# cbg-ethz/metMHN

Measured on AMD Instinct MI355X. Metric: full-cohort log-lik+grad evals/sec at n=20 events; kronvec HBM GB/s, higher is better.
Workload: dtype f64

## Files before the change

metmhn_amd/csrc/engine.hip:

```cpp
#include <hip/hip_runtime.h>
#include <rccl/rccl.h>
#include <dlfcn.h>

#include <algorithm>
#include <chrono>
#include <cmath>
#include <cstdio>
#include <cstdlib>
#include <cstring>
#include <string>
#include <vector>

#include "../../include/metmhn_amd.h"
#include "kernels.h"
#include "tsolve.h"
#include "small.h"
#include "wsolve.h"
#include "wclass.h"
#include "sampler.h"

namespace mmhn {

static thread_local std::string g_err;

struct Fail {
  std::string msg;
};
#define HIPCHECK(expr)                                                                       \
  do {                                                                                       \
    hipError_t e_ = (expr);                                                                  \
    if (e_ != hipSuccess)                                                                    \
      throw Fail{std::string(#expr) + ": " + hipGetErrorString(e_) + " (" + __FILE__ + ":" + \
                 std::to_string(__LINE__) + ")"};                                            \
  } while (0)
#define REQUIRE(cond, text) \
  do {                      \
    if (!(cond)) throw Fail{std::string(text)}; \
  } while (0)

template <typename U>
struct DevArr {
  U* p = nullptr;
  size_t n = 0;
  void alloc(size_t count) {
    if (count <= n && p) return;
    release();
    if (count == 0) return;
    HIPCHECK(hipMalloc(reinterpret_cast<void**>(&p), count * sizeof(U)));
    n = count;
  }
  void release() {
    if (p) (void)hipFree(p);
    p = nullptr;
    n = 0;
  }
  ~DevArr() { release(); }
  DevArr() = default;
  DevArr(const DevArr&) = delete;
  DevArr& operator=(const DevArr&) = delete;
  DevArr(DevArr&& o) noexcept : p(o.p), n(o.n) { o.p = nullptr; o.n = 0; }
  DevArr& operator=(DevArr&& o) noexcept {
    if (this != &o) { release(); p = o.p; n = o.n; o.p = nullptr; o.n = 0; }
    return *this;
  }
};

struct CList {
  std::vector<CItem> items;
  std::vector<int> deps;
  DevArr<CItem> d_items;
  DevArr<int> d_deps;
  int maxk = 0;
  int nlevels = 0;
  void clear() { items.clear(); deps.clear(); maxk = 0; nlevels = 0; }
};
enum Route : uint8_t { RT_W = 0, RT_P = 1, RT_T = 2 };

struct Staged {
  std::vector<int> pats, paired, probs;
  DevArr<int> d_pats, d_paired, d_probs;
  std::vector<int2> map, lmap;
  std::vector<int> lof;
  DevArr<int2> d_map, d_lmap;
  DevArr<int2> d_grc;
  CList cl[2];
  int maxk = 0;
  bool kind2 = false;
  bool empty() const { return pats.empty(); }
};

struct Batch {
  std::vector<PatRec> pats;
  std::vector<Desc> dJ, dS;
  std::vector<int2> mapJ, mapS;
  long long vecJ = 0, vecS = 0, asize = 0, tabJ = 0, tabS = 0;
  int id = 0;
  int maxkJ = 0, maxkS = 0;
  int maxkcJ = 0;
  bool has_kind2 = false;
  std::vector<int2> lmapJ, lmapS;
  std::vector<int> lofJ, lofS;
  std::vector<int2> mapX;
  DevArr<int2> d_mapX;
  DevArr<int2> d_grc[4];
  DevArr<int2> d_grcJ;
  std::vector<int> sp_list[3][SP_NCLASS];
  DevArr<int> d_sp_list[3][SP_NCLASS];
  bool has_small = false;
  int mk1p = 9;
  Staged stg[2];
  std::vector<int> paired;
  DevArr<int> d_paired;
  std::vector<uint8_t> route;
  std::vector<int> olist;
  DevArr<int> d_olist;
  bool wpath = false;
  bool wdirect = false;
  std::vector<WDesc> wd;
  DevArr<WDesc> d_wd;
  int wnx = -1;
  std::vector<WChain> wchains;
  DevArr<WChain> d_wchains;
  long long offT = 0;
  CList clJ[2];
  std::vector<int2> lmapT;
  std::vector<int> lofT;
  DevArr<int2> d_lmapT;
  int maxkT = 0, maxkP = 0;
  int max_dl = 0;
  std::vector<int> ptoff;
  std::vector<uint32_t> ptiles;
  DevArr<int> d_ptoff;
  DevArr<uint32_t> d_ptiles;
  double seeded_bytes_P = 0;
  std::vector<int4> pcl;
  DevArr<int4> d_pcl;
  DevArr<PatRec> d_pats;
  DevArr<Desc> d_dJ, d_dS;
  DevArr<int2> d_mapJ, d_mapS, d_lmapJ, d_lmapS;
};

static bool dead_tile(const Desc& d, uint32_t H) {
  if (d.mode != JOINT || d.seedbit < TB) return false;
  const uint32_t xhi = H << TB, hmask = ~((1u << TB) - 1u);
  if (xhi & (1u << d.seedbit)) return false;
  if (xhi & d.lone & hmask) return true;
  const uint32_t pp = d.pairP & hmask & ~(1u << 31);
  const uint32_t pm = (pp << 1);
  if (((xhi & pp) << 1) != (xhi & pm)) return true;
  return false;
}

static void build_levels(const std::vector<int2>& map, const std::vector<Desc>* descs, bool prune,
                         std::vector<int2>& lmap, std::vector<int>& lof) {
  int maxl = 0;
  std::vector<int2> keep;
  keep.reserve(map.size());
  for (const int2& m : map) {
    if (prune && descs && dead_tile((*descs)[m.x], (uint32_t)m.y)) continue;
    keep.push_back(m);
    maxl = std::max(maxl, popc((uint32_t)m.y));
  }
  lof.assign(maxl + 2, 0);
  for (const int2& m : keep) lof[popc((uint32_t)m.y) + 1]++;
  for (int l = 0; l <= maxl; ++l) lof[l + 1] += lof[l];
  lmap.resize(keep.size());
  std::vector<int> cur(lof.begin(), lof.end() - 1);
  for (const int2& m : keep) lmap[cur[popc((uint32_t)m.y)]++] = m;
}

static inline long long a_size(const Desc& d) {
  const int kP = popc(d.maskP), kM = popc(d.maskM), kE = popc(d.pairP);
  return ((long long)(kP + 1) << kP) + ((long long)(kM + 1) << kM) + ((long long)(kE + 2) << kE);
}

static void add_tiles(std::vector<int2>& map, int prob, int k) {
  const int tiles = k > TB ? 1 << (k - TB) : 1;
  for (int t = 0; t < tiles; ++t) map.push_back(make_int2(prob, t));
// ... 152 lines not shown
    double v;
    if (e == 0) v = em[0];
    else if (e == 1) v = nm[0];
    else if (e == 2) v = n_em;
    else if (e == 3) v = n_pat;
    else {
      int q = e - 4;
      if (q < NN) v = em[1 + q];
      else if ((q -= NN) < NN) v = nm[1 + q];
      else if ((q -= NN) < N) v = em[1 + NN + q];
      else if ((q -= N) < N) v = nm[1 + NN + q];
      else v = em[1 + NN + N + (q - N)];
    }
    o[e] = v;
  }
}

__global__ void k_pack_wsums(const double* __restrict__ sums, int N, double w, double* __restrict__ o, double flag) {
  const int st = 1 + N * N + 2 * N, NN = N * N;
  if (blockIdx.x == 0 && threadIdx.x == 0) o[st] = flag;
  const double* em = sums;
  const double* nm = sums + st;
  for (int e = blockIdx.x * blockDim.x + threadIdx.x; e < st; e += gridDim.x * blockDim.x)
    o[e] = e < 1 + NN + N ? w * em[e] + nm[e] : w * em[e];
}

__global__ void k_copy_words(const uint4* __restrict__ src, uint4* __restrict__ dst, int n) {
  const int i = blockIdx.x * blockDim.x + threadIdx.x;
  if (i < n) dst[i] = src[i];
}
__global__ void k_begin_eval(const uint4* __restrict__ src, uint4* __restrict__ dst, int n, double* __restrict__ sums, int nsums,
                             uint4* __restrict__ z, long long nz) {
  const long long i0 = (long long)blockIdx.x * blockDim.x + threadIdx.x, step = (long long)gridDim.x * blockDim.x;
  if (i0 < n) dst[i0] = src[i0];
  if (i0 < nsums) sums[i0] = 0.0;
  for (long long i = i0; i < nz; i += step) z[i] = uint4{0u, 0u, 0u, 0u};
}

__global__ __launch_bounds__(BLOCK) void k_reduce_parts_pack(const double* __restrict__ part, int stride, int nelem, int nchunk,
                                                             double* sums, int mode, int N, double a, double b,
                                                             double* __restrict__ o) {
  const int e = blockIdx.x * BLOCK + threadIdx.x;
  if (e == 0 && mode == 2) o[stride] = b;
  if (e >= stride) return;
  double em = sums[e], nm = sums[stride + e];
  if (e < nelem) {
    double acc0 = 0, acc1 = 0;
#pragma unroll 8
    for (int c = 0; c < nchunk; ++c) {
      acc0 += part[((long long)c * 2 + 0) * stride + e];
      acc1 += part[((long long)c * 2 + 1) * stride + e];
    }
    em += acc0; nm += acc1;
    sums[e] = em; sums[stride + e] = nm;
  }
  const int NN = N * N;
  if (mode == 2) { o[e] = e < 1 + NN + N ? a * em + nm : a * em; return; }
  if (e == 0) { o[0] = em; o[1] = nm; o[2] = a; o[3] = b; }
  else if (e < 1 + NN) { o[4 + (e - 1)] = em; o[4 + NN + (e - 1)] = nm; }
  else if (e < 1 + NN + N) { o[4 + 2 * NN + (e - 1 - NN)] = em; o[4 + 2 * NN + N + (e - 1 - NN)] = nm; }
  else o[4 + 2 * NN + 2 * N + (e - 1 - NN - N)] = em;
}

template <typename T>
struct Engine : EngineBase {
  int n = 0, N = 0;
  size_t ws_limit = 0;
  DevArr<Params<T>> d_par;
  Params<T>* h_par = nullptr;
  double* h_abi = nullptr;
  void* h_par_dev = nullptr;
  double* h_abi_dev = nullptr;
  bool zero_copy = true;
  bool time_kernels = true;
  std::vector<int8_t> dat;
  long long n_pat = 0;
  int n_cols = 0;
  std::vector<Batch> batches;
  double n_em = 0;
  DevArr<T> pi, lidgJ, qJ, rhsJ, rhsS, pS, lidgS, qS, seedS, GS, dots, bmJ, bmS, tabJ, tabS;
  DevArr<T> zarena;
  struct View { T* p = nullptr; } GJ, DJ, Abuf;
  static long long zarena_elems(long long nJ, long long asize, int N) { return up4(3 * nJ * N * N) + up4(3 * nJ * N) + up4(asize); }
  static long long up4(long long v) { return (v + 3) / 4 * 4; }
  int pi_owner = -1, qJ_owner = -1;
  DevArr<double> lp, out, sums, abi_sums, redbuf;
  DevArr<JLink<T>> links;
  ncclComm_t comm = nullptr;
  int comm_rank = 0, comm_size = 1;
  DevArr<uint16_t> d_perm;
  DevArr<int> d_lvl;
  bool use_jacobi = false;
  bool poison = false;
  hipStream_t side[3] = {};
  hipEvent_t ev_fork[3] = {}, ev_join[3] = {};
  bool small_path = true;
  int prep_split_max = 2048;
  int psolve_min = 384;
  int wsolve_min = 128;
  bool force_timing = false;
  bool coop_fault = false;
  int pcl_per = 16;
  int coop_wgs = 0;
  bool coop = true;
  DevArr<CoopCtl> coop_ctl;
  DevArr<unsigned> coop_flags[2];
  unsigned coop_epoch = 0;
  int coop_slot = 0;
  int cur_lane = 0;
  unsigned* h_abort = nullptr;
  unsigned* h_abort_dev = nullptr;
  int wsolve_wgs = 0;
  int wsolve_mode = 1;
  DevArr<T> piM, qM;
  int n_cu = 256;
  mmhn_counters cnt{};
  std::vector<std::pair<hipEvent_t, hipEvent_t>> ev_pool;
  size_t ev_used = 0;
  std::vector<double> ev_bytes;
  std::vector<int> ev_slot;

  Engine(int dev, int n_mut) : n(n_mut), N(n_mut + 1) {
    device = dev;
    cnt.comm_rank = -1;
    REQUIRE(n_mut >= 1 && n_mut < MAXN, "n_mut must be in [1, 31]");
    DevGuard guard(device);
    HIPCHECK(hipStreamCreateWithFlags(&stream, hipStreamNonBlocking));
    d_par.alloc(NPSET);
    HIPCHECK(hipHostMalloc(reinterpret_cast<void**>(&h_par), NPSET * sizeof(Params<T>), hipHostMallocDefault));
    HIPCHECK(hipHostGetDevicePointer(&h_par_dev, h_par, 0));
    static_assert(sizeof(Params<T>) % sizeof(uint4) == 0, "parameter block: whole 16-byte words");
    sums.alloc(2 * stride());
    size_t free_b = 0, total_b = 0;
    HIPCHECK(hipMemGetInfo(&free_b, &total_b));
    ws_limit = (size_t)(0.7 * (double)free_b);
    {
      std::vector<uint16_t> perm((size_t)(TB + 1) << TB, 0);
      std::vector<int> lvl((size_t)(TB + 1) * (TB + 2), 0);
      for (int t = 0; t <= TB; ++t) {
        int pos = 0;
        for (int l = 0; l <= t; ++l) {
          lvl[(size_t)t * (TB + 2) + l] = pos;
          for (uint32_t x = 0; x < (1u << t); ++x)
            if (popc(x) == l) perm[((size_t)t << TB) + pos++] = (uint16_t)x;
        }
        lvl[(size_t)t * (TB + 2) + t + 1] = pos;
      }
      d_perm.alloc(perm.size());
      d_lvl.alloc(lvl.size());
      HIPCHECK(hipMemcpy(d_perm.p, perm.data(), perm.size() * sizeof(uint16_t), hipMemcpyHostToDevice));
      HIPCHECK(hipMemcpy(d_lvl.p, lvl.data(), lvl.size() * sizeof(int), hipMemcpyHostToDevice));
      const char* sv = std::getenv("MMHN_SOLVER");
      use_jacobi = sv && std::string(sv) == "jacobi";
      if (const char* pm = std::getenv("MMHN_PSOLVE_MIN")) { psolve_min = std::atoi(pm); wsolve_min = psolve_min; }
      if (const char* pm = std::getenv("MMHN_WSOLVE_MIN")) wsolve_min = std::atoi(pm);
      if (const char* pm = std::getenv("MMHN_COOP")) coop = std::atoi(pm) != 0;
      if (const char* pm = std::getenv("MMHN_TIME_KERNELS")) force_timing = std::atoi(pm) != 0;
      if (const char* pm = std::getenv("MMHN_COOP_WGS")) coop_wgs = std::atoi(pm);
      if (const char* pm = std::getenv("MMHN_PCL_PER")) pcl_per = std::max(1, std::atoi(pm));
      if (const char* pm = std::getenv("MMHN_COOP_FAULT")) coop_fault = std::atoi(pm) != 0;
      if (const char* po = std::getenv("MMHN_POISON")) poison = std::atoi(po) != 0;
      if (const char* sp = std::getenv("MMHN_SMALL")) small_path = std::atoi(sp) != 0;
      if (const char* sp = std::getenv("MMHN_ZEROCOPY")) zero_copy = std::atoi(sp) != 0;
      if (const char* sp = std::getenv("MMHN_PREP_SPLIT")) prep_split_max = std::atoi(sp);
      if (const char* ms = std::getenv("MMHN_WSOLVE")) wsolve_mode = std::atoi(ms);
      if (const char* ms = std::getenv("MMHN_WSOLVE_WGS")) wsolve_wgs = std::atoi(ms);
// ... 633 lines not shown
          }
        }
        auto item_tiles = [&](const int4& it) -> long long {
          if (it.y == 2) return 0;
          const Desc& dj = b.dJ[it.x];
          const int kc = popc(it.y == 0 ? dj.maskP : dj.maskM);
          return (long long)(it.w - it.z) << (kc > PCA ? kc - PCA : 0);
        };
        std::stable_sort(b.pcl.begin(), b.pcl.end(), [&](const int4& x, const int4& y) { return item_tiles(x) > item_tiles(y); });
        up(b.d_pcl, b.pcl);
      }
      build_levels(b.mapS, nullptr, false, b.lmapS, b.lofS);
      b.paired.clear();
      for (size_t pi_ = 0; pi_ < b.pats.size(); ++pi_) if (b.pats[pi_].j >= 0) b.paired.push_back((int)pi_);
      up(b.d_paired, b.paired);
      for (int w = 0; w < 3; ++w) for (int c = 0; c < SP_NCLASS; ++c) b.sp_list[w][c].clear();
      for (int w = 0; w < 2; ++w) { Staged& g = b.stg[w]; g.pats.clear(); g.paired.clear(); g.probs.clear(); g.kind2 = false; }
      bool class_fits[SP_NCLASS];
      for (int c = 0; c < SP_NCLASS; ++c)
        class_fits[c] = (spatient_lds<T>(N, spatient_class_maxk(c)) + 15) / 16 * 16 * (size_t)(c == 0 ? SP_PPB0 : c == 1 ? 2 : 1) + 64 <= (size_t)160 * 1024;
      const bool all_staged = !small_path || use_jacobi;
      for (size_t pi_ = 0; pi_ < b.pats.size(); ++pi_) {
        const PatRec& pr = b.pats[pi_];
        int ks = -1;
        for (int part = 0; part < 2; ++part) if (pr.s[part] >= 0) ks = std::max(ks, b.dS[pr.s[part]].k);
        if (ks < 0) continue;
        int c = 0;
        while (c < SP_NCLASS - 1 && ks > spatient_class_maxk(c)) ++c;
        if (all_staged || ks > TB || !class_fits[c]) {
          Staged& g = b.stg[all_staged || pr.j >= 0 ? 1 : 0];
          g.pats.push_back((int)pi_);
          if (pr.j >= 0) g.paired.push_back((int)pi_);
          for (int part = 0; part < 2; ++part) if (pr.s[part] >= 0) g.probs.push_back(pr.s[part]);
          if (pr.kind == 2) g.kind2 = true;
          continue;
        }
        const bool side_by_side = pr.j >= 0 && pr.s[0] >= 0 && pr.s[1] >= 0 && c < 2;
        b.sp_list[side_by_side ? 2 : pr.j >= 0 ? 1 : 0][c].push_back((int)pi_);
      }
      b.mk1p = spatient_class_maxk(1);
      if (!b.sp_list[1][2].empty() && b.sp_list[1][2].size() <= 16) {
        int mk = 0;
        for (int pi_ : b.sp_list[1][2])
          for (int part = 0; part < 2; ++part) if (b.pats[pi_].s[part] >= 0) mk = std::max(mk, b.dS[b.pats[pi_].s[part]].k);
        if (mk <= 10 && (spatient_lds<T>(N, mk) + 15) / 16 * 16 * 2 + 64 <= (size_t)160 * 1024) {
          for (int pi_ : b.sp_list[1][2]) b.sp_list[b.pats[pi_].s[0] >= 0 && b.pats[pi_].s[1] >= 0 ? 2 : 1][1].push_back(pi_);
          b.sp_list[1][2].clear();
          b.mk1p = mk;
        }
      }
      {
        auto ksize = [&](int pi_) {
          const PatRec& pr = b.pats[pi_];
          int ks = 0;
          for (int part = 0; part < 2; ++part) if (pr.s[part] >= 0) ks = std::max(ks, 64 * b.dS[pr.s[part]].k + (pr.s[0] >= 0 && pr.s[1] >= 0 ? 32 : 0) + pr.kind);
          return ks;
        };
        for (int w = 0; w < 3; ++w)
          for (int c = 0; c < SP_NCLASS; ++c)
            std::stable_sort(b.sp_list[w][c].begin(), b.sp_list[w][c].end(), [&](int x, int y) { return ksize(x) > ksize(y); });
      }
      b.has_small = false;
      for (int w = 0; w < 3; ++w)
        for (int c = 0; c < SP_NCLASS; ++c) {
          if (!b.sp_list[w][c].empty()) b.has_small = true;
          up(b.d_sp_list[w][c], b.sp_list[w][c]);
        }
      for (int w = 0; w < 2; ++w) {
        Staged& g = b.stg[w];
        std::vector<char> isg(b.dS.size(), 0);
        for (int sp : g.probs) isg[sp] = 1;
        g.map.clear(); g.maxk = 0;
        for (const int2& m : b.mapS) if (isg[m.x]) { g.map.push_back(m); g.maxk = std::max(g.maxk, b.dS[m.x].k); }
        build_levels(g.map, nullptr, false, g.lmap, g.lof);
        g.cl[0].clear(); g.cl[1].clear();
        if (!use_jacobi && g.lof.size() > 2) { build_clist(g.map, b.dS, false, false, g.cl[0]); build_clist(g.map, b.dS, false, true, g.cl[1]); }
        up(g.d_pats, g.pats); up(g.d_paired, g.paired); up(g.d_probs, g.probs);
        up(g.d_map, g.map); up(g.d_lmap, g.lmap);
        std::vector<int2> gc;
        for (const int2& e : grad_chunks(b.dS, GK_S)) if (isg[e.x]) gc.push_back(e);
        up(g.d_grc, gc);
      }
      b.wdirect = b.wpath && wsolve_mode != 2;
      for (Desc& dj : b.dJ) dj.wl = -1;
      if (b.wdirect) for (size_t i = 0; i < b.wd.size(); ++i) b.dJ[b.wd[i].prob].wl = (int)i;
      up(b.d_dJ, b.dJ); up(b.d_dS, b.dS); up(b.d_mapJ, b.mapJ); up(b.d_mapS, b.mapS);
      up(b.d_lmapJ, b.lmapJ); up(b.d_lmapS, b.lmapS);
      up(b.d_ptoff, b.ptoff); up(b.d_ptiles, b.ptiles); up(b.d_mapX, b.mapX);
      {
        std::vector<int2> all;
        for (int kd = 0; kd < 4; ++kd) {
          std::vector<int2> gc = grad_chunks(kd == GK_S ? b.dS : b.dJ, kd);
          up(b.d_grc[kd], gc);
          if (kd != GK_S) for (int2 e : gc) all.push_back(int2{e.x, e.y | (kd << 24)});
        }
        up(b.d_grcJ, all);
      }
      mvJ = std::max(mvJ, b.vecJ); mvS = std::max(mvS, b.vecS);
      mZ = std::max<size_t>(mZ, (size_t)zarena_elems((long long)b.dJ.size(), b.asize, N));
      mtJ = std::max(mtJ, b.tabJ); mtS = std::max(mtS, b.tabS);
      if (b.wpath && !b.wdirect) mvM = std::max(mvM, b.vecJ);
      mnJ = std::max(mnJ, b.dJ.size()); mnS = std::max(mnS, b.dS.size()); mp = std::max(mp, b.pats.size());
    }
    pi.alloc(mvJ); qJ.alloc(mvJ);
    piM.alloc(mvM); qM.alloc(mvM);
    if (use_jacobi) { lidgJ.alloc(mvJ); rhsJ.alloc(mvJ); }
    links.alloc(std::max<size_t>(mnJ, 1));
    tabJ.alloc(mtJ); tabS.alloc(mtS);
    pi_owner = qJ_owner = -1;
    rhsS.alloc(mvS); pS.alloc(mvS); lidgS.alloc(mvS); qS.alloc(mvS);
    seedS.alloc(mnS);
    GS.alloc(mnS * N * N); zarena.alloc(mZ);
    dots.alloc(2 * mp); bmJ.alloc(mnJ * 64); bmS.alloc(mnS * 64);
    lp.alloc(mp); out.alloc(mp * stride()); redbuf.alloc(((mp + red_per((int)mp) - 1) / red_per((int)mp)) * 2 * (size_t)stride());
  }

  bool small_forked[2] = {false, false}, fork_recorded[2] = {false, false};
  void small_fork(int which) {
    HIPCHECK(hipEventRecord(ev_fork[which], stream));
    fork_recorded[which] = true;
  }
  void small_classes(const Batch& b, int which, bool grad) {
    const int n0 = (int)b.sp_list[which][0].size(), n1 = (int)b.sp_list[which][1].size(), n2 = (int)b.sp_list[which][2].size();
    const int np0 = which ? (int)b.sp_list[2][0].size() : 0, np1 = which ? (int)b.sp_list[2][1].size() : 0;
    const int mk0 = spatient_class_maxk(0), mk1 = which ? b.mk1p : spatient_class_maxk(1), mk2 = spatient_class_maxk(2);
    const bool on_side = which == 0 ? (n0 + n1 + n2 > 0) : n2 > 0;
    hipStream_t sd = side[which];
    if (on_side) {
      if (!fork_recorded[which]) HIPCHECK(hipEventRecord(ev_fork[which], stream));
      HIPCHECK(hipStreamWaitEvent(sd, ev_fork[which], 0));
    }
    fork_recorded[which] = false;
#define SP_TAIL b.d_pats.p, b.d_dS.p, d_par.p, d_perm.p, d_lvl.p, b.d_dJ.p, b.d_wd.p, pi.p, links.p, pS.p, qS.p, GS.p, bmS.p, dots.p, lp.p
    auto big_class = [&]() {
      if (!n2) return;
      const size_t lds = (spatient_lds<T>(N, mk2) + 15) / 16 * 16;
      hipLaunchKernelGGL((k_spatient<T, 1024, 1>), dim3(n2), dim3(1024), lds, sd, b.d_sp_list[which][2].p, n2, SP_TAIL, mk2, N, grad ? 1 : 0);
      HIPCHECK(hipGetLastError());
    };
    big_class();
    if (n0 + n1 + np0 + np1) {
      const size_t s0 = (spatient_lds<T>(N, mk0) + 15) / 16 * 16, s1 = (spatient_lds<T>(N, mk1) + 15) / 16 * 16;
      const size_t lds = std::max(s0 * SP_PPB0, n1 + np1 ? s1 * (np1 ? 2 : 1) : 0) + 64;
      const int nblk = (n0 + SP_PPB0 - 1) / SP_PPB0 + n1 + (np0 + SP_PPB0 / 2 - 1) / (SP_PPB0 / 2) + np1;
      hipLaunchKernelGGL((k_spatient2<T>), dim3(nblk), dim3(256), lds, which == 0 ? sd : stream,
                         b.d_sp_list[which][0].p, n0, mk0, b.d_sp_list[which][1].p, n1, mk1,
                         b.d_sp_list[2][0].p, np0, b.d_sp_list[2][1].p, np1, SP_TAIL, N, grad ? 1 : 0);
      HIPCHECK(hipGetLastError());
    }
#undef SP_TAIL
    if (on_side) HIPCHECK(hipEventRecord(ev_join[which], sd));
    small_forked[which] = on_side;
  }
  void small_join(int which) {
    if (small_forked[which]) HIPCHECK(hipStreamWaitEvent(stream, ev_join[which], 0));
    small_forked[which] = false;
  }

  void evaluate(const double* lt, const double* ldp, const double* ldm, bool grad, double* host_sums,
                double* host_out) {
    REQUIRE(!sums_pending, "an evaluation begun with mmhn_cohort_sums_begin has not been collected");
    auto t0 = std::chrono::steady_clock::now();
    const int st = stride();
    small_forked[0] = small_forked[1] = fork_recorded[0] = fork_recorded[1] = false;
    bool head_done = false;
    if (zero_copy && !batches.empty()) {
      build_params(lt, ldp, ldm, false);
      const Batch& b0 = batches.front();
      long long nz = grad && !b0.dJ.empty() ? zarena_elems((long long)b0.dJ.size(), b0.asize, N) * (long long)sizeof(T) / 16 : 0;
      const bool fill_here = nz <= (32ll << 20) / 16;
      if (!fill_here) nz = 0;
      const int nw = (int)(NPSET * sizeof(Params<T>) / sizeof(uint4));
      const long long need = std::max<long long>(std::max<long long>(nw, 2 * st), nz);
      const int nblk = (int)std::min<long long>((need + 255) / 256, 4096);
      hipLaunchKernelGGL(k_begin_eval, dim3(nblk), dim3(256), 0, stream, static_cast<const uint4*>(h_par_dev),
                         reinterpret_cast<uint4*>(d_par.p), nw, sums.p, 2 * st, reinterpret_cast<uint4*>(zarena.p), nz);
      HIPCHECK(hipGetLastError());
      head_done = fill_here;
    } else {
      build_params(lt, ldp, ldm);
      HIPCHECK(hipMemsetAsync(sums.p, 0, 2 * st * sizeof(double), stream));
    }
    for (Batch& b : batches) {
      const int npat = (int)b.pats.size(), nJ = (int)b.dJ.size(), nS = (int)b.dS.size();
      const int tJ = (int)b.mapJ.size();
      const PList LJ{b.d_dJ.p, b.d_mapJ.p, tJ, b.maxkJ, b.vecJ, b.d_lmapJ.p, &b.lofJ, tabJ.p};
      const bool fused_small = b.has_small, staged = !b.stg[0].empty() || !b.stg[1].empty();
      coop_alone = b.stg[0].empty();
      auto staged_fwd = [&](const Staged& g) {
        if (g.empty()) return;
        const int nG = (int)g.pats.size(), tG = (int)g.map.size();
        const PList LG{b.d_dS.p, g.d_map.p, tG, g.maxk, b.vecS, g.d_lmap.p, &g.lof, tabS.p, g.cl};
        hipLaunchKernelGGL((k_staged_init<T>), dim3(nG), dim3(BLOCK), 0, stream, b.d_pats.p, b.d_dS.p, rhsS.p, GS.p, bmS.p, N, grad ? 1 : 0, g.d_pats.p);
        HIPCHECK(hipGetLastError());
        if (g.probs.size() >= 256)
          hipLaunchKernelGGL((k_prep<T, false, 1024>), dim3((unsigned)g.probs.size()), dim3(1024), prep_lds<T>(N), stream, b.d_dS.p, d_par.p, tabS.p, g.d_probs.p);
        else
          hipLaunchKernelGGL((k_prep<T, false>), dim3((unsigned)g.probs.size()), dim3(BLOCK), prep_lds<T>(N), stream, b.d_dS.p, d_par.p, tabS.p, g.d_probs.p);
        HIPCHECK(hipGetLastError());
        if (!g.paired.empty()) {
          hipLaunchKernelGGL((k_gather_marg<T>), dim3((unsigned)g.paired.size(), 2, g.maxk > 10 ? 8 : 1), dim3(BLOCK), 0, stream,
                             b.d_pats.p, b.d_dJ.p, b.d_dS.p, d_par.p, pi.p, rhsS.p, links.p, g.d_paired.p, b.d_wd.p);
          HIPCHECK(hipGetLastError());
        }
        launch_diag(b.d_dS.p, g.d_map.p, tG, nullptr, lidgS.p, nullptr, KD_LIDG);
        solve(false, LG, pS.p, lidgS.p, rhsS.p, 0, nullptr);
        hipLaunchKernelGGL((k_seeds<T>), dim3((nG + 255) / 256), dim3(256), 0, stream, b.d_pats.p, nG, b.d_dS.p,
                           d_par.p, pS.p, seedS.p, lp.p, g.d_pats.p);
        HIPCHECK(hipGetLastError());
      };
      auto staged_adj = [&](const Staged& g) {
        if (g.empty()) return;
        const int tG = (int)g.map.size();
        const PList LG{b.d_dS.p, g.d_map.p, tG, g.maxk, b.vecS, g.d_lmap.p, &g.lof, tabS.p, g.cl};
        solve(true, LG, qS.p, lidgS.p, nullptr, 1, seedS.p);
        launch_grad_rows(b.d_dS.p, (int)g.probs.size(), g.maxk, nullptr, pS.p, qS.p, GS.p, GK_S, g.d_grc);
        if (g.kind2) {
          hipLaunchKernelGGL((k_bit_marg<T>), dim3(tG), dim3(BLOCK), 0, stream, b.d_dS.p, g.d_map.p, d_par.p, pS.p, qS.p, bmS.p);
          HIPCHECK(hipGetLastError());
        }
      };
      time_kernels = force_timing || b.vecJ + b.vecS >= (1ll << 26);
      const long long gjs = (long long)nJ * N * N;
      GJ.p = zarena.p;
      DJ.p = GJ.p + up4(3 * gjs);
      Abuf.p = DJ.p + up4(3ll * nJ * N);
      if (grad && nJ && !(head_done && &b == &batches.front())) zero(zarena.p, zarena_elems(nJ, b.asize, N));
      prep(b.d_dJ.p, nJ, tabJ.p, true, b.maxkcJ);
      bool own_forked = false;
      if (!b.stg[0].empty() && !time_kernels) {
        HIPCHECK(hipEventRecord(ev_fork[2], stream));
        HIPCHECK(hipStreamWaitEvent(side[2], ev_fork[2], 0));
        hipStream_t keep = stream;
        stream = side[2]; cur_lane = 1;
        try {
          staged_fwd(b.stg[0]);
          if (grad) staged_adj(b.stg[0]);
        } catch (...) { stream = keep; cur_lane = 0; throw; }
        stream = keep; cur_lane = 0;
        HIPCHECK(hipEventRecord(ev_join[2], side[2]));
        own_forked = true;
      }
      if (fused_small) small_fork(0);
      if (!use_jacobi && nJ) {
        if (pi_owner != b.id) { zero(pi.p + b.offT, b.vecJ - b.offT); pi_owner = b.id; }
        if (grad && qJ_owner != b.id) { zero(qJ.p + b.offT, b.vecJ - b.offT); qJ_owner = b.id; }
        if (poison && b.offT > 0) {
          HIPCHECK(hipMemsetAsync(pi.p, 0xFF, (size_t)b.offT * sizeof(T), stream));
          if (grad) HIPCHECK(hipMemsetAsync(qJ.p, 0xFF, (size_t)b.offT * sizeof(T), stream));
        }
      }
      if (use_jacobi) {
        launch_diag(b.d_dJ.p, b.d_mapJ.p, tJ, nullptr, lidgJ.p, nullptr, KD_LIDG);
        solve(false, LJ, pi.p, lidgJ.p, nullptr, 2, nullptr);
      } else {
        psolve(false, b, pi.p, 2);
      }
      if (fused_small) small_classes(b, 0, grad);
      if (fused_small) small_classes(b, 1, grad);
      if (!own_forked) staged_fwd(b.stg[0]);
      staged_fwd(b.stg[1]);
      if (grad) {
        if (!own_forked) staged_adj(b.stg[0]);
        staged_adj(b.stg[1]);
        small_join(1);
        if (nJ) {
          if (use_jacobi) zero(rhsJ.p, b.vecJ);
          for (int part = 0; part < 2 && !b.stg[1].paired.empty(); ++part) {
            if (b.stg[1].paired.size() >= 256)
              hipLaunchKernelGGL((k_scatter_marg<T, 1024>), dim3((unsigned)b.stg[1].paired.size()), dim3(1024), 0, stream, b.d_pats.p, b.d_dJ.p,
                                 b.d_dS.p, d_par.p, qS.p, rhsS.p, use_jacobi ? rhsJ.p : nullptr, dots.p, part, b.stg[1].d_paired.p);
            else
            hipLaunchKernelGGL((k_scatter_marg<T>), dim3((unsigned)b.stg[1].paired.size()), dim3(BLOCK), 0, stream, b.d_pats.p, b.d_dJ.p,
                               b.d_dS.p, d_par.p, qS.p, rhsS.p, use_jacobi ? rhsJ.p : nullptr, dots.p, part, b.stg[1].d_paired.p);
            HIPCHECK(hipGetLastError());
          }
          if (use_jacobi) solve(true, LJ, qJ.p, lidgJ.p, rhsJ.p, 0, nullptr);
          else psolve(true, b, qJ.p, 3);
          if (!use_jacobi) {
            const double mbytes = (double)b.vecJ * sizeof(T);
            timed(MMHN_K_PCLASS, mbytes, [&]() {
              if (b.wdirect) {
                const int nW = (int)b.wd.size();
                hipLaunchKernelGGL((k_wclass<T>), dim3((unsigned)std::min(nW, n_cu)), dim3(WROWS), wclass_lds<T>(), stream, b.d_dJ.p, b.d_wd.p, nW, pi.p, qJ.p, Abuf.p);
              }
              if (!b.pcl.empty())
                hipLaunchKernelGGL((k_pclass<T, true>), dim3((unsigned)b.pcl.size()), dim3(CMB), PC_LDS_ELEMS * sizeof(T), stream, b.d_dJ.p, b.d_wd.p, pi.p, qJ.p, Abuf.p, b.d_pcl.p);
              else if ((int)b.wd.size() < nJ || !b.wdirect)
                hipLaunchKernelGGL((k_pclass<T, false>), dim3(nJ), dim3(CMB), PC_LDS_ELEMS * sizeof(T), stream, b.d_dJ.p, b.d_wd.p, pi.p, qJ.p, Abuf.p);
            });
            if (!b.mapX.empty())
              hipLaunchKernelGGL((k_class_marg<T>), dim3((unsigned)b.mapX.size()), dim3(CMB), 2 * sizeof(T) << TB, stream,
                                 b.d_dJ.p, b.d_mapX.p, pi.p, qJ.p, Abuf.p);
          } else {
            hipLaunchKernelGGL((k_class_marg<T>), dim3(tJ), dim3(CMB), 2 * sizeof(T) << TB, stream, b.d_dJ.p,
                               b.d_mapJ.p, pi.p, qJ.p, Abuf.p);
          }
          HIPCHECK(hipGetLastError());
          if (b.pcl.empty()) {
            hipLaunchKernelGGL((k_eq_flows<T>), dim3(nJ), dim3(BLOCK), 0, stream, b.d_dJ.p, b.d_wd.p, pi.p, qJ.p, Abuf.p);
            HIPCHECK(hipGetLastError());
          }
          launch_grad_rows(b.d_dJ.p, nJ, b.maxkcJ, Abuf.p, nullptr, nullptr, GJ.p, -1, b.d_grcJ, DJ.p, gjs);
        }
      }
      if (fused_small) { small_join(0); small_join(1); }
      if (own_forked) HIPCHECK(hipStreamWaitEvent(stream, ev_join[2], 0));
      const AsmArgs<T> aa{b.d_pats.p, b.d_dJ.p, b.d_dS.p, d_par.p, GS.p, GJ.p, gjs, dots.p, DJ.p, (long long)nJ * N, bmS.p, lp.p, N,
                          grad ? 1 : 0};
      const int nelem = grad ? st : 1;
// ... 1141 lines not shown
```

metmhn_amd/csrc/wclass.h:

```cpp
#pragma once
#include "kernels.h"

namespace mmhn {

template <typename T>
struct WClass {
  static constexpr int CHE = 32768 / (int)sizeof(T);
  static constexpr size_t lds = 4 * (size_t)CHE * sizeof(T) + 64;
};
template <typename T>
constexpr size_t wclass_lds() { return WClass<T>::lds; }

template <typename T>
__global__ __launch_bounds__(WROWS) void k_wclass(const Desc* __restrict__ descs, const WDesc* __restrict__ wds, int nw,
                                                  const T* __restrict__ p, const T* __restrict__ q, T* A) {
  using C = WCfg<T>;
  constexpr int RB = C::RB, HB = C::HB, NC = 1 << RB, H = 1 << HB, KC = C::KC, WNXR = C::KR - WTB;
  constexpr int QE = 16 / (int)sizeof(T), LGQ = QE == 2 ? 1 : 2, NQ = NC / QE;
  constexpr int CHE = WClass<T>::CHE;
  typedef T VecT __attribute__((ext_vector_type(NC)));
  typedef T QT __attribute__((ext_vector_type(QE)));
  static_assert(NQ == 2 && CHE == WROWS * NC, "a block row is two 16-byte pieces; a block fills one staged array");
  extern __shared__ __align__(16) unsigned char smem[];
  T* const lds = reinterpret_cast<T*>(smem);
  const int tid = threadIdx.x;
  const uint32_t rho = wrho((uint32_t)tid >> 6, (uint32_t)tid & 63u);
  for (int it = blockIdx.x; it < nw; it += gridDim.x) {
    const WDesc& wd = wds[it];
    const Desc& d = descs[wd.prob];
    const int k = d.k, kR = wd.kR, kC = wd.kC, nXc = wd.nXc, nXr = wd.nXr;
    const bool majP = wd.majP != 0;
    const long long half = 1ll << (k - 1);
    const T* ps = p + d.off + half;
    const T* qs = q + d.off + half;
    const int kP = __popc(d.maskP);
    T* outR = A + d.aoff + (majP ? 0 : class_block_size(kP));
    T* outC = A + d.aoff + (majP ? class_block_size(kP) : 0);
    const int NBc = (1 << nXc) << HB;
    auto ldv = [&](const T* src, uint32_t Sigma, uint32_t beta, uint32_t row) -> VecT {
      const QT* a = reinterpret_cast<const QT*>(src + wpos<T>(Sigma, beta, row, 0));
      const QT lo = a[0], hi = a[1];
      VecT v;
#pragma unroll
      for (int e = 0; e < QE; ++e) { v[e] = lo[e]; v[QE + e] = hi[e]; }
      return v;
    };
    auto dot = [&](const VecT& a, const VecT& b) -> T {
      T s = a[0] * b[0];
#pragma unroll
      for (int c = 1; c < NC; ++c) s += a[c] * b[c];
      return s;
    };
    __syncthreads();
    for (uint32_t Sx = 0; Sx < (1u << nXr); ++Sx) {
      T acc[1 + WTB + WNXR];
#pragma unroll
      for (int s = 0; s < 1 + WTB + WNXR; ++s) acc[s] = T(0);
      VecT pn = ldv(ps, Sx << nXc, 0, rho), qn = ldv(qs, Sx << nXc, 0, rho);
      for (int B = 0; B < NBc; ++B) {
        const uint32_t Sigma = ((uint32_t)B >> HB) | (Sx << nXc), beta = (uint32_t)B & (uint32_t)(H - 1);
        const VecT pv = pn, qv = qn;
        if (B + 1 < NBc) {
          const uint32_t Sg2 = ((uint32_t)(B + 1) >> HB) | (Sx << nXc), b2 = (uint32_t)(B + 1) & (uint32_t)(H - 1);
          pn = ldv(ps, Sg2, b2, rho); qn = ldv(qs, Sg2, b2, rho);
        }
        T* qb = lds + (B & 1) * CHE;
        {
          QT lo, hi;
#pragma unroll
          for (int e = 0; e < QE; ++e) { lo[e] = qv[e]; hi[e] = qv[QE + e]; }
          *reinterpret_cast<QT*>(qb + (size_t)tid * QE) = lo;
          *reinterpret_cast<QT*>(qb + (size_t)(WROWS + tid) * QE) = hi;
        }
        __syncthreads();
        acc[0] -= dot(pv, qv);
#pragma unroll
        for (int i = 0; i < WTB; ++i) {
          const uint32_t nb = (uint32_t)tid | (1u << i);
          const QT lo = *reinterpret_cast<const QT*>(qb + (size_t)nb * QE);
          const QT hi = *reinterpret_cast<const QT*>(qb + (size_t)(WROWS + nb) * QE);
          T s = T(0);
#pragma unroll
          for (int e = 0; e < QE; ++e) s += pv[e] * lo[e] + pv[QE + e] * hi[e];
          acc[1 + i] += s;
        }
#pragma unroll
        for (int i = 0; i < WNXR; ++i) {
          if (i < nXr && !((Sx >> i) & 1u)) {
            const VecT qx = ldv(qs, Sigma | (1u << (nXc + i)), beta, rho);
            acc[1 + WTB + i] += dot(pv, qx);
          }
        }
      }
      const long long S = (long long)tid | ((long long)Sx << WTB);
      outR[S] = acc[0];
#pragma unroll
      for (int i = 0; i < WTB; ++i)
        if (!((tid >> i) & 1)) outR[((long long)(1 + i) << kR) + S] = acc[1 + i];
#pragma unroll
      for (int i = 0; i < WNXR; ++i)
        if (i < nXr && !((Sx >> i) & 1u)) outR[((long long)(1 + WTB + i) << kR) + S] = acc[1 + WTB + i];
    }
    {
      const int NPc = (1 << kC) / QE;
      const int RCH = CHE >> kC;
      const int nch = WROWS / RCH;
      const int cp = tid & (NPc - 1);
      const int r0 = tid / NPc, rstep = WROWS / NPc;
      T ac[QE][1 + KC];
#pragma unroll
      for (int e = 0; e < QE; ++e)
#pragma unroll
        for (int s = 0; s <= KC; ++s) ac[e][s] = T(0);
      const int rl = RCH * NQ;
      auto piece_src = [&](int g, uint32_t Sx, int ch) -> long long {
        const int run = g / rl, rr = g % rl;
        const uint32_t Sigma = ((uint32_t)run >> HB) | (Sx << nXc), beta = (uint32_t)run & (uint32_t)(H - 1);
        return wpos<T>(Sigma, beta, (uint32_t)(ch * RCH + (rr >> 1)), (uint32_t)((rr & 1) * QE));
      };
      auto piece_dst = [&](int g) -> int {
        const int run = g / rl, rr = g % rl;
        return ((rr >> 1) << kC) + (run << RB) + (rr & 1) * QE;
      };
      const int ntot = nch << nXr;
      QT rp[2], rq[2];
      auto fetch = [&](int cidx) {
        const uint32_t Sx = (uint32_t)(cidx / nch);
        const int ch = cidx % nch;
#pragma unroll
        for (int j = 0; j < 2; ++j) {
          const long long src = piece_src(tid + WROWS * j, Sx, ch);
          rp[j] = *reinterpret_cast<const QT*>(ps + src);
          rq[j] = *reinterpret_cast<const QT*>(qs + src);
        }
      };
      __syncthreads();
      fetch(0);
      for (int cidx = 0; cidx < ntot; ++cidx) {
        T* pc = lds + (size_t)(2 * (cidx & 1)) * CHE;
        T* qc = pc + CHE;
#pragma unroll
        for (int j = 0; j < 2; ++j) {
          const int dst = piece_dst(tid + WROWS * j);
          *reinterpret_cast<QT*>(pc + dst) = rp[j];
          *reinterpret_cast<QT*>(qc + dst) = rq[j];
        }
        if (cidx + 1 < ntot) fetch(cidx + 1);
        __syncthreads();
        for (int r = r0; r < RCH; r += rstep) {
          const T* prow = pc + ((size_t)r << kC);
          const T* qrow = qc + ((size_t)r << kC);
          const QT pv = *reinterpret_cast<const QT*>(prow + cp * QE);
          const QT qv = *reinterpret_cast<const QT*>(qrow + cp * QE);
#pragma unroll
          for (int e = 0; e < QE; ++e) ac[e][0] -= pv[e] * qv[e];
#pragma unroll
          for (int b = 0; b < LGQ; ++b)
#pragma unroll
            for (int e = 0; e < QE; ++e)
              if (!((e >> b) & 1)) ac[e][1 + b] += pv[e] * qv[e | (1 << b)];
#pragma unroll
          for (int b = LGQ; b < KC; ++b) {
            if (b < kC) {
              const QT nq = *reinterpret_cast<const QT*>(qrow + (cp | (1 << (b - LGQ))) * QE);
#pragma unroll
              for (int e = 0; e < QE; ++e) ac[e][1 + b] += pv[e] * nq[e];
            }
          }
        }
      }
      __syncthreads();
      T* red = lds;
#pragma unroll
      for (int s = 0; s <= KC; ++s) {
#pragma unroll
        for (int e = 0; e < QE; ++e) {
          if (s <= kC) {
            red[tid] = ac[e][s];
            __syncthreads();
            if (tid < NPc) {
              T v = T(0);
              for (int g = 0; g < rstep; ++g) v += red[tid + g * NPc];
              const uint32_t Tc = (uint32_t)(tid * QE + e);
              if (s == 0 || !((Tc >> (s - 1)) & 1u)) outC[((long long)s << kC) + Tc] = v;
            }
            __syncthreads();
          }
        }
      }
    }
  }
}

}
```

Baseline: 21.45.

## Compute low cross-row partner terms from LDS chunks in W-class column pass

New measurement: 22.05 (median of 6 runs). 2.8% higher.

```diff
diff --git a/metmhn_amd/csrc/engine.hip b/metmhn_amd/csrc/engine.hip
--- a/metmhn_amd/csrc/engine.hip
+++ b/metmhn_amd/csrc/engine.hip
@@ -94,6 +94,7 @@
   std::vector<Desc> dJ, dS;
   std::vector<int2> mapJ, mapS;
   long long vecJ = 0, vecS = 0, asize = 0, tabJ = 0, tabS = 0;
+  long long aclr = 0;
   int id = 0;
   int maxkJ = 0, maxkS = 0;
   int maxkcJ = 0;
@@ -412,6 +413,7 @@
   DevArr<T> zarena;
   struct View { T* p = nullptr; } GJ, DJ, Abuf;
   static long long zarena_elems(long long nJ, long long asize, int N) { return up4(3 * nJ * N * N) + up4(3 * nJ * N) + up4(asize); }
+  static long long zclear_elems(const Batch& b, int N) { return zarena_elems((long long)b.dJ.size(), b.aclr, N); }
   static long long up4(long long v) { return (v + 3) / 4 * 4; }
   int pi_owner = -1, qJ_owner = -1;
   DevArr<double> lp, out, sums, abi_sums, redbuf;
@@ -1211,6 +1213,14 @@
         up(g.d_grc, gc);
       }
       b.wdirect = b.wpath && wsolve_mode != 2;
+      {
+        long long ao = 0;
+        for (int pj = 0; pj < nJ; ++pj) if (!(b.wdirect && b.route[pj] == RT_W)) { b.dJ[pj].aoff = ao; ao += a_size(b.dJ[pj]); }
+        b.aclr = up4(ao);
+        ao = b.aclr;
+        for (int pj = 0; pj < nJ; ++pj) if (b.wdirect && b.route[pj] == RT_W) { b.dJ[pj].aoff = ao; ao += a_size(b.dJ[pj]); }
+        b.asize = ao;
+      }
       for (Desc& dj : b.dJ) dj.wl = -1;
       if (b.wdirect) for (size_t i = 0; i < b.wd.size(); ++i) b.dJ[b.wd[i].prob].wl = (int)i;
       up(b.d_dJ, b.dJ); up(b.d_dS, b.dS); up(b.d_mapJ, b.mapJ); up(b.d_mapS, b.mapS);
@@ -1296,7 +1306,7 @@
     if (zero_copy && !batches.empty()) {
       build_params(lt, ldp, ldm, false);
       const Batch& b0 = batches.front();
-      long long nz = grad && !b0.dJ.empty() ? zarena_elems((long long)b0.dJ.size(), b0.asize, N) * (long long)sizeof(T) / 16 : 0;
+      long long nz = grad && !b0.dJ.empty() ? zclear_elems(b0, N) * (long long)sizeof(T) / 16 : 0;
       const bool fill_here = nz <= (32ll << 20) / 16;
       if (!fill_here) nz = 0;
       const int nw = (int)(NPSET * sizeof(Params<T>) / sizeof(uint4));
@@ -1354,7 +1364,8 @@
       GJ.p = zarena.p;
       DJ.p = GJ.p + up4(3 * gjs);
       Abuf.p = DJ.p + up4(3ll * nJ * N);
-      if (grad && nJ && !(head_done && &b == &batches.front())) zero(zarena.p, zarena_elems(nJ, b.asize, N));
+      if (grad && nJ && !(head_done && &b == &batches.front())) zero(zarena.p, zclear_elems(b, N));
+      if (grad && nJ && poison) poison_fill(Abuf.p + b.aclr, b.asize - b.aclr);
       prep(b.d_dJ.p, nJ, tabJ.p, true, b.maxkcJ);
       bool own_forked = false;
       if (!b.stg[0].empty() && !time_kernels) {
diff --git a/metmhn_amd/csrc/wclass.h b/metmhn_amd/csrc/wclass.h
--- a/metmhn_amd/csrc/wclass.h
+++ b/metmhn_amd/csrc/wclass.h
@@ -6,8 +6,29 @@
 template <typename T>
 struct WClass {
   static constexpr int CHE = 32768 / (int)sizeof(T);
-  static constexpr size_t lds = 4 * (size_t)CHE * sizeof(T) + 64;
+  static constexpr int LGCHE = sizeof(T) == 8 ? 12 : 13;
+  static constexpr int LGMINR = 2;
+  static constexpr int MX = WCfg<T>::KR - WTB < LGCHE - LGMINR - WCfg<T>::RB - WCfg<T>::HB ? WCfg<T>::KR - WTB
+                                                                                           : LGCHE - LGMINR - WCfg<T>::RB - WCfg<T>::HB;
+  static constexpr int XP = MX * (CHE >> (WCfg<T>::RB + WCfg<T>::HB));
+  static constexpr size_t lds = (4 * (size_t)CHE + 2 * (size_t)XP) * sizeof(T) + WROWS * sizeof(uint16_t) + 64;
+  static_assert((1 << LGCHE) == CHE, "");
 };
+template <typename T>
+__host__ __device__ inline int wclass_mbits(int kC, int nXr) {
+  const int m = WClass<T>::LGCHE - WClass<T>::LGMINR - kC;
+  return m < 0 ? 0 : m < nXr ? m : nXr;
+}
+template <typename T>
+__device__ __forceinline__ T seg_sum(T v, int lg) {
+  if (lg > 0) v = dpp_stage<0>(v);
+  if (lg > 1) v = dpp_stage<1>(v);
+  if (lg > 2) v = dpp_stage<2>(v);
+  if (lg > 3) v = dpp_stage<3>(v);
+  if (lg > 4) v = dpp_stage<4>(v);
+  if (lg > 5) v = dpp_stage<5>(v);
+  return v;
+}
 template <typename T>
 constexpr size_t wclass_lds() { return WClass<T>::lds; }
 
@@ -25,6 +46,8 @@
   T* const lds = reinterpret_cast<T*>(smem);
   const int tid = threadIdx.x;
   const uint32_t rho = wrho((uint32_t)tid >> 6, (uint32_t)tid & 63u);
+  uint16_t* const rinv = reinterpret_cast<uint16_t*>(lds + 4 * (size_t)CHE + 2 * (size_t)WClass<T>::XP);
+  rinv[rho] = (uint16_t)tid;
   for (int it = blockIdx.x; it < nw; it += gridDim.x) {
     const WDesc& wd = wds[it];
     const Desc& d = descs[wd.prob];
@@ -37,6 +60,7 @@
     T* outR = A + d.aoff + (majP ? 0 : class_block_size(kP));
     T* outC = A + d.aoff + (majP ? class_block_size(kP) : 0);
     const int NBc = (1 << nXc) << HB;
+    const int mX = wclass_mbits<T>(kC, nXr);
     auto ldv = [&](const T* src, uint32_t Sigma, uint32_t beta, uint32_t row) -> VecT {
       const QT* a = reinterpret_cast<const QT*>(src + wpos<T>(Sigma, beta, row, 0));
       const QT lo = a[0], hi = a[1];
@@ -86,7 +110,7 @@
         }
 #pragma unroll
         for (int i = 0; i < WNXR; ++i) {
-          if (i < nXr && !((Sx >> i) & 1u)) {
+          if (i >= mX && i < nXr && !((Sx >> i) & 1u)) {
             const VecT qx = ldv(qs, Sigma | (1u << (nXc + i)), beta, rho);
             acc[1 + WTB + i] += dot(pv, qx);
           }
@@ -99,37 +123,58 @@
         if (!((tid >> i) & 1)) outR[((long long)(1 + i) << kR) + S] = acc[1 + i];
 #pragma unroll
       for (int i = 0; i < WNXR; ++i)
-        if (i < nXr && !((Sx >> i) & 1u)) outR[((long long)(1 + WTB + i) << kR) + S] = acc[1 + WTB + i];
+        if (i >= mX && i < nXr && !((Sx >> i) & 1u)) outR[((long long)(1 + WTB + i) << kR) + S] = acc[1 + WTB + i];
     }
     {
-      const int NPc = (1 << kC) / QE;
-      const int RCH = CHE >> kC;
-      const int nch = WROWS / RCH;
+      constexpr int XP = WClass<T>::XP, JU = sizeof(T) == 8 ? 2 : 1;
+      static_assert(CHE == 2 * WROWS * QE, "a thread takes two rows of a chunk");
+      const int lgR = WClass<T>::LGCHE - kC - mX;
+      const int RCH = 1 << lgR, RCX = RCH << mX;
+      const int lgnch = WTB - lgR, nch = 1 << lgnch;
+      const int lgP = kC - LGQ, NPc = 1 << lgP;
       const int cp = tid & (NPc - 1);
-      const int r0 = tid / NPc, rstep = WROWS / NPc;
+      const int r0 = tid >> lgP, rstep = WROWS >> lgP;
+      const int lgRX = lgR + mX, nW = lgP > 6 ? 1 << (lgP - 6) : 1;
+      T* const xpart = lds + 4 * (size_t)CHE;
       T ac[QE][1 + KC];
 #pragma unroll
       for (int e = 0; e < QE; ++e)
 #pragma unroll
         for (int s = 0; s <= KC; ++s) ac[e][s] = T(0);
-      const int rl = RCH * NQ;
-      auto piece_src = [&](int g, uint32_t Sx, int ch) -> long long {
-        const int run = g / rl, rr = g % rl;
-        const uint32_t Sigma = ((uint32_t)run >> HB) | (Sx << nXc), beta = (uint32_t)run & (uint32_t)(H - 1);
+      const int lgrl = lgR + 1;
+      auto piece_src = [&](int g, uint32_t sxh, int ch) -> long long {
+        const int run = g >> lgrl, rr = g & ((1 << lgrl) - 1);
+        const uint32_t Sigma = ((uint32_t)run >> HB) | (sxh << (nXc + mX)), beta = (uint32_t)run & (uint32_t)(H - 1);
         return wpos<T>(Sigma, beta, (uint32_t)(ch * RCH + (rr >> 1)), (uint32_t)((rr & 1) * QE));
       };
       auto piece_dst = [&](int g) -> int {
-        const int run = g / rl, rr = g % rl;
-        return ((rr >> 1) << kC) + (run << RB) + (rr & 1) * QE;
-      };
-      const int ntot = nch << nXr;
+        const int run = g >> lgrl, rr = g & ((1 << lgrl) - 1);
+        const int sxl = run >> (kC - RB), cb = run & ((1 << (kC - RB)) - 1);
+        return (((sxl << lgR) | (rr >> 1)) << kC) + (cb << RB) + (rr & 1) * QE;
+      };
+      auto row_S = [&](int cidx, int r) -> long long {
+        const uint32_t Sx = (uint32_t)(r >> lgR) | ((uint32_t)(cidx >> lgnch) << mX);
+        return (long long)rinv[((cidx & (nch - 1)) << lgR) | (r & (RCH - 1))] | ((long long)Sx << WTB);
+      };
+      auto xfinish = [&](int cidx) {
+        const T* xp = xpart + (cidx & 1) * XP;
+        for (int i = tid; i < (mX << lgRX); i += WROWS) {
+          const int l = i >> lgRX, r = i & (RCX - 1);
+          if (!((r >> (lgR + l)) & 1)) {
+            T v = xp[(size_t)i * nW];
+            for (int w = 1; w < nW; ++w) v += xp[(size_t)i * nW + w];
+            outR[((long long)(1 + WTB + l) << kR) + row_S(cidx, r)] = v;
+          }
+        }
+      };
+      const int ntot = nch << (nXr - mX);
       QT rp[2], rq[2];
       auto fetch = [&](int cidx) {
-        const uint32_t Sx = (uint32_t)(cidx / nch);
-        const int ch = cidx % nch;
+        const uint32_t sxh = (uint32_t)(cidx >> lgnch);
+        const int ch = cidx & (nch - 1);
 #pragma unroll
         for (int j = 0; j < 2; ++j) {
-          const long long src = piece_src(tid + WROWS * j, Sx, ch);
+          const long long src = piece_src(tid + WROWS * j, sxh, ch);
           rp[j] = *reinterpret_cast<const QT*>(ps + src);
           rq[j] = *reinterpret_cast<const QT*>(qs + src);
         }
@@ -147,7 +192,10 @@
         }
         if (cidx + 1 < ntot) fetch(cidx + 1);
         __syncthreads();
-        for (int r = r0; r < RCH; r += rstep) {
+        if (mX > 0 && cidx > 0) xfinish(cidx - 1);
+#pragma unroll JU
+        for (int j = 0; j < 2; ++j) {
+          const int r = r0 + j * rstep;
           const T* prow = pc + ((size_t)r << kC);
           const T* qrow = qc + ((size_t)r << kC);
           const QT pv = *reinterpret_cast<const QT*>(prow + cp * QE);
@@ -167,9 +215,20 @@
               for (int e = 0; e < QE; ++e) ac[e][1 + b] += pv[e] * nq[e];
             }
           }
+#pragma unroll 1
+          for (int l = 0; l < mX; ++l) {
+            const QT nq = *reinterpret_cast<const QT*>(qc + ((size_t)(r | (RCH << l)) << kC) + cp * QE);
+            T s = pv[0] * nq[0];
+#pragma unroll
+            for (int e = 1; e < QE; ++e) s += pv[e] * nq[e];
+            s = seg_sum(s, lgP < 6 ? lgP : 6);
+            if ((cp & 63) == ((NPc - 1) & 63))
+              xpart[(cidx & 1) * XP + (size_t)((l << lgRX) + r) * nW + (cp >> 6)] = s;
+          }
         }
       }
       __syncthreads();
+      if (mX > 0) xfinish(ntot - 1);
       T* red = lds;
 #pragma unroll
       for (int s = 0; s <= KC; ++s) {
```
